# moritzmeister/hops-examples

Hardware: AMD Instinct MI355X
Metric: images/sec MNIST CNN + steps/sec Chicago-taxi DNN at 1/2/4/8 MI355X (higher is better)
Workload: dtype bf16; 1 GPU; model=MNIST CNN (experiment.mirrored model, 1394282 params), Adadelta(1.0), global_batch=32, per_gpu_batch=32, parallelism=dp1, engine=PersistentMnistStep, hipgraph=False, steps_per_execution=32, warmup_steps_run=5

## Files before the change

csrc/ops/mnist_persist.hip:

```cpp
#include "common.h"
#include "mnist_cnn.h"
#include "optim_core.h"
#include "wg_prims.h"

namespace mnistp {
using namespace wgp;
using namespace mnist_cnn;

constexpr int B = 32;
constexpr int NCONV = C2 * 128 + C2 + C1 * 4 + C1;
constexpr int OFF_B2 = C2 * 128, OFF_W1 = OFF_B2 + C2, OFF_B1 = OFF_W1 + C1 * 4;
constexpr int SLICE = 52, NSLICE = (NCONV + SLICE - 1) / SLICE;
constexpr int NRED = 19;
constexpr int NHEAD = B;
constexpr int GRID = NPOS + NHEAD;
constexpr int PAY = 272;
constexpr int PAY_DH = 0, PAY_H = 128, PAY_DL = 256, PAY_LOSS = 268, PAY_COR = 269;
constexpr int FL_A = 0, FL_B = 256, FL_C = 512, FL_D = 768, FL_WORDS = 1024;
constexpr int FL_EPOCH = FL_WORDS - 2;
constexpr int D_F32 = OFF_B2 * 2;
constexpr int D_BYTES = D_F32 + (NCONV - OFF_B2) * 4;
constexpr int TGB_N = NHEAD * (HID / 2);
constexpr int TG_WORDS = 2 * 2 * TGB_N;
static_assert(FL_WORDS % 2 == 0 && TGB_N % 256 == 0, "granules are 8-B aligned; every thread owns TGB_N / 256");

constexpr int DHS = row_stride(HID), DCS = row_stride(4 * B);
static_assert(DHS == 136 && DCS == 136, "strides the kernel was tuned with");

constexpr int L_W1 = 0;
constexpr int L_W2 = L_W1 + HID * W1S * 2;
constexpr int L_CW1 = L_W2 + C2 * W2S * 2;
constexpr int L_CB1 = L_CW1 + C1 * 4 * 4;
constexpr int L_CB2 = L_CB1 + C1 * 4;
constexpr int L_XIN = L_CB2 + C2 * 4;
constexpr int L_C1 = L_XIN + B * 16 * 4;
constexpr int L_POOL = L_C1 + B * 9 * C1S * 2;
constexpr int L_AM = L_POOL + B * PLS * 2;
constexpr int L_DH = L_AM + B * C2;
constexpr int L_DC2 = L_DH + B * DHS * 2;
constexpr int L_STG = L_DC2 + C2 * DCS * 2;
constexpr int L_RED = L_STG + NCONV * 4;
constexpr int L_SL = L_RED + 1024 * 4;
constexpr int L_KEEP = L_SL + 3 * 64 * 4;
constexpr int LDS_BYTES = L_KEEP + B * C2;

constexpr int H_W2 = 0;
constexpr int H_B2 = H_W2 + 3 * NCLS * HID * 4;
constexpr int H_B1 = H_B2 + 3 * 16 * 4;
constexpr int H_RED = H_B1 + 3 * HID * 4;
constexpr int H_H = H_RED + 8 * HID * 4;
constexpr int H_LOG = H_H + HID * 4;
constexpr int H_PAY = H_LOG + 16 * 4;
constexpr int H_ALL = H_PAY + PAY * 4;
constexpr int H_END = H_ALL + NHEAD * PAY * 4;
constexpr int H_DHS = H_END;
static_assert(H_DHS + B * DHS * 2 <= LDS_BYTES, "head LDS map must fit the position map");

constexpr int XMAX = 8;
constexpr long XS_POOL = (long)NPOS * 4 * 64 * 16;
constexpr long XS_DHT = 8L * 64 * 16;
constexpr int NFC2 = NCLS * HID + HID + NCLS, NFC2P = 1424;
constexpr long XS_FC2 = NFC2P * 4;
constexpr long XS_CONV = (long)NSLICE * SLICE * 4;
constexpr long XO_POOL = 0, XO_DHT = XO_POOL + 2L * XMAX * XS_POOL, XO_FC2 = XO_DHT + 2L * XMAX * XS_DHT,
               XO_CONV = XO_FC2 + 2L * XMAX * XS_FC2, X_BYTES = XO_CONV + 2L * XMAX * XS_CONV;
constexpr int XF_POOL = 0, XF_H = XMAX * NPOS, XF_CONV = XF_H + XMAX, XF_WORDS = XF_CONV + XMAX * NSLICE;
static_assert(NFC2 <= NFC2P && NFC2P % 4 == 0 && X_BYTES < 0x7fffffffL, "exchange geometry");
static_assert(LDS_BYTES <= 160 * 1024, "one workgroup per CU: 160 KiB LDS");
static_assert(L_RED + NRED * SLICE * 4 <= L_SL && 2 * 32 * 5 * 4 <= 1024 * 4, "reduce scratch");
static_assert(NRED * 13 <= 256 && NSLICE * SLICE >= NCONV && NSLICE <= NPOS, "slice geometry");

struct Args {
  float* master;
  bf16_raw* shadow;
  float* s1;
  float* s2;
  long off[8];
  const unsigned char* xs;
  const long long* ys;
  long nbatch;
  long long* cursor;
  unsigned long long* rng;
  float* step_dev;
  const float* hp_dev;
  float* slabA;
  float* slabB;
  float* slabC;
  float* slabD;
  unsigned* flags;
  unsigned* err;
  float* out;
  unsigned long long* dbg;
  OptHP hp;
  float drop_p, xscale, xshift;
  unsigned salt;
  int nsteps;
  int acquire;
  long long tmo;
  long long tmo0;
  int pollw, stagger;
  int pollw_a, pollw_b, pollw_c, pollw_d;
  int head1w;
  int hand;
  float inv_gb;
  int world, rank;
  int loopback;
  int xfence;
  long long* xstep;
  unsigned char* xbuf[XMAX];
  unsigned* xflag[XMAX];
};


__device__ __forceinline__ int xslot(const Args& a, int peer) { return a.loopback ? peer : a.rank; }

__device__ __forceinline__ bool wait_all(const unsigned* flags, int n, unsigned epoch, unsigned* err, unsigned code,
                                      int acquire, int* s_ok, long long tmo, int pollw = 1, int stagger = 0,
                                      int poll1 = 0) {
  if (pollw <= 1) {
    if (threadIdx.x < 64) {
      const int lane = threadIdx.x;
      int good = 1;
      const long long t0 = wall_clock64();
      for (unsigned spins = 0;; ++spins) {
        int ok = 1;
        unsigned e = poll1 ? flag_load(err) : 0u;
        for (int k = lane; k < n; k += 64) ok &= flag_load(flags + k) == epoch;
        if (__all(ok)) break;
        if (!poll1) e = flag_load(err);
        if (__builtin_amdgcn_readfirstlane(e) != 0u) {
          good = 0;
          break;
        }
        if ((spins & 15u) == 15u && wall_clock64() - t0 > tmo) {
          if (lane == 0) atomicCAS(err, 0u, code);
          good = 0;
          break;
        }
        __builtin_amdgcn_s_sleep(1);
      }
      if (acquire && good) __builtin_amdgcn_fence(__ATOMIC_ACQUIRE, "agent");
      drain();
      if (lane == 0) *s_ok = good;
    }
    __syncthreads();
    const int g = *s_ok;
    return g != 0;
  }
  volatile int* gen = s_ok + 1;
  const int wave = threadIdx.x >> 6;
  if (wave < pollw) {
    const int lane = threadIdx.x & 63;
    int good = 1;
    for (int d = 0; d < wave * stagger && __builtin_amdgcn_readfirstlane(*gen) != (int)code; ++d)
      __builtin_amdgcn_s_sleep(1);
    const long long t0 = wall_clock64();
    for (unsigned spins = 0;; ++spins) {
      if (__builtin_amdgcn_readfirstlane(*gen) == (int)code) break;
      int ok = 1;
      unsigned e = poll1 ? flag_load(err) : 0u;
      for (int k = lane; k < n; k += 64) ok &= flag_load(flags + k) == epoch;
      if (__all(ok)) {
        if (lane == 0) {
          s_ok[0] = 1;
          *gen = (int)code;
        }
        break;
      }
      if (!poll1) e = flag_load(err);
      if (__builtin_amdgcn_readfirstlane(e) != 0u) good = 0;
      if ((spins & 15u) == 15u && wall_clock64() - t0 > tmo) {
        if (lane == 0) atomicCAS(err, 0u, code);
        good = 0;
      }
      if (!good) {
        if (lane == 0) {
          s_ok[0] = 0;
          *gen = (int)code;
        }
        break;
      }
      __builtin_amdgcn_s_sleep(1);
    }
    if (acquire) __builtin_amdgcn_fence(__ATOMIC_ACQUIRE, "agent");
    drain();
  }
  __syncthreads();
  const int g = s_ok[0];
  return g != 0;
}

__device__ __forceinline__ bool wait_peers(const Args& a, int base, int stride, unsigned epoch, unsigned code,
                                        int* s_ok) {
  if (threadIdx.x < 64) {
    const int lane = threadIdx.x;
    const unsigned* page = a.xflag[a.rank];
    int good = 1;
    const long long t0 = wall_clock64();
    for (unsigned spins = 0;; ++spins) {
      const bool mine = lane < a.world && lane != a.rank;
      unsigned e = (a.hand & 2) ? flag_load(a.err) : 0u;
      const int ok = !mine || (int)(xflag_load(page + base + lane * stride) - epoch) >= 0;
      if (__all(ok)) break;
      if (!(a.hand & 2)) e = flag_load(a.err);
      if (__builtin_amdgcn_readfirstlane(e) != 0u) {
        good = 0;
        break;
      }
      if ((spins & 15u) == 15u && wall_clock64() - t0 > a.tmo) {
        if (lane == 0) atomicCAS(a.err, 0u, code);
        good = 0;
        break;
      }
      __builtin_amdgcn_s_sleep(1);
    }
    drain();
    if (lane == 0) *s_ok = good;
  }
  __syncthreads();
  const int g = *s_ok;
  return g != 0;
}
__device__ __forceinline__ void raise_peers(const Args& a, int base, int stride, unsigned epoch) {
// ... 460 lines not shown
      for (int j = 0; j < 8; ++j) acc[j] = (f32x4){0.f, 0.f, 0.f, 0.f};
      const bf16_raw* cb = C1 + (2 * fq * 9 + (tq >> 1) * 3 + (tq & 1)) * C1S + 4 * tp;
      bf16x8 af[2], bfr[2][8];
      auto cfrag = [&](int kk, int st) {
#pragma unroll
        for (int j = 0; j < 8; ++j) {
          const int t = j >> 1;
          const bf16_raw* q = cb + (kk * 8 * 9 + (t >> 1) * 3 + (t & 1)) * C1S + (j & 1) * 16;
          bfr[st][j] = lds_tr(q, q + 9 * C1S);
        }
      };
      auto afrag = [&](int kk, int st) { af[st] = lds8(DC2 + (w * 16 + fr) * DCS + kk * 32 + fq * 8); };
      cfrag(0, 0);
      __syncthreads();
      stamp(a, s, 4);
      afrag(0, 0);
#pragma unroll
      for (int kk = 0; kk < 4; ++kk) {
        if (kk + 1 < 4) {
          afrag(kk + 1, (kk + 1) & 1);
          cfrag(kk + 1, (kk + 1) & 1);
        }
        __builtin_amdgcn_sched_barrier(0);
#pragma unroll
        for (int j = 0; j < 8; ++j) acc[j] = mma32(af[kk & 1], bfr[kk & 1][j], acc[j]);
      }
#pragma unroll
      for (int j = 0; j < 8; ++j)
#pragma unroll
        for (int r = 0; r < 4; ++r) STG[(w * 16 + fq * 4 + r) * 128 + j * 16 + fr] = acc[j][r];
    }
    {
      const int mh = w >> 1, h = w & 1, ci = h * 16 + fr;
      bf16x8 af[2][4], bfr[2][4];
#pragma unroll
      for (int kk = 0; kk < 2; ++kk) {
        const int k1 = kk * 32 + 8 * fq + tq;
#pragma unroll
        for (int i = 0; i < 4; ++i) {
          const int m0 = (mh * 4 + i) * 16 + 4 * tp;
          af[kk][i] = lds_tr(DC2 + k1 * DCS + m0, DC2 + (k1 + 4) * DCS + m0);
        }
#pragma unroll
        for (int t = 0; t < 4; ++t) {
          const int c0 = (2 * t + h) * 16 + 4 * tp;
          bfr[kk][t] = lds_tr(W2 + k1 * W2S + c0, W2 + (k1 + 4) * W2S + c0);
        }
      }
      __syncthreads();
      {
        const auto R = rsrc(a.slabC + ((long)par * NPOS + p) * NCONV);
        constexpr int NK = OFF_B2 / 4 / 256;
        f32x4 v[NK];
#pragma unroll
        for (int k = 0; k < NK; ++k) v[k] = *(const f32x4*)(STG + (tid + 256 * k) * 4);
        __builtin_amdgcn_sched_barrier(0);
#pragma unroll
        for (int k = 0; k < NK; ++k) bst16<SC1>(R, (tid + 256 * k) * 16, v[k]);
      }
      f32x4 acc[4][4];
#pragma unroll
      for (int i = 0; i < 4; ++i)
#pragma unroll
        for (int t = 0; t < 4; ++t) acc[i][t] = (f32x4){0.f, 0.f, 0.f, 0.f};
#pragma unroll
      for (int kk = 0; kk < 2; ++kk)
#pragma unroll
        for (int t = 0; t < 4; ++t)
#pragma unroll
          for (int i = 0; i < 4; ++i) acc[i][t] = mma32(af[kk][i], bfr[kk][t], acc[i][t]);
      bf16_raw c1v[4][9];
#pragma unroll
      for (int i = 0; i < 4; ++i)
#pragma unroll
        for (int pos = 0; pos < 9; ++pos) c1v[i][pos] = C1[((4 * (mh * 4 + i) + fq) * 9 + pos) * C1S + ci];
      if constexpr (!DP) {
        bf16x8 wa[2], wb[4];
#pragma unroll
        for (int ii = 0; ii < 2; ++ii) {
          const int n0 = (2 * w + ii) * 16 + 4 * tp;
          wa[ii] = lds_tr(DH + (8 * fq + tq) * DHS + n0, DH + (8 * fq + tq + 4) * DHS + n0);
        }
#pragma unroll
        for (int j = 0; j < 4; ++j) {
          const int c0 = j * 16 + 4 * tp;
          wb[j] = lds_tr(POOL + (8 * fq + tq) * PLS + c0, POOL + (8 * fq + tq + 4) * PLS + c0);
        }
#pragma unroll
        for (int ii = 0; ii < 2; ++ii)
#pragma unroll
          for (int j = 0; j < 4; ++j) gw[ii][j] = mma32(wa[ii], wb[j], (f32x4){0.f, 0.f, 0.f, 0.f});
      }
      float gk[5] = {0.f, 0.f, 0.f, 0.f, 0.f};
      f32x4 xq[2][4];
#pragma unroll
      for (int c = 0; c < 4; ++c) xq[0][c] = *(const f32x4*)(XIN + (4 * (mh * 4) + fq) * 16 + 4 * c);
#pragma unroll
      for (int i = 0; i < 4; ++i) {
        if (i + 1 < 4) {
#pragma unroll
          for (int c = 0; c < 4; ++c) xq[(i + 1) & 1][c] = *(const f32x4*)(XIN + (4 * (mh * 4 + i + 1) + fq) * 16 + 4 * c);
        }
        float d[9];
#pragma unroll
        for (int k = 0; k < 9; ++k) d[k] = 0.f;
#pragma unroll
        for (int t = 0; t < 4; ++t)
#pragma unroll
          for (int q = 0; q < 4; ++q) d[((q >> 1) + (t >> 1)) * 3 + (q & 1) + (t & 1)] += acc[i][t][q];
        const f32x4* xi = xq[i & 1];
#pragma unroll
        for (int py = 0; py < 3; ++py)
#pragma unroll
          for (int px = 0; px < 3; ++px) {
            const int pos = py * 3 + px;
            const float dd = (short)c1v[i][pos] > 0 ? d[pos] : 0.f;
            gk[0] = fmaf(dd, xi[py][px], gk[0]);
            gk[1] = fmaf(dd, xi[py][px + 1], gk[1]);
            gk[2] = fmaf(dd, xi[py + 1][px], gk[2]);
            gk[3] = fmaf(dd, xi[py + 1][px + 1], gk[3]);
            gk[4] += dd;
          }
      }
#pragma unroll
      for (int k = 0; k < 5; ++k) {
        gk[k] += __shfl_xor(gk[k], 16, 64);
        gk[k] += __shfl_xor(gk[k], 32, 64);
      }
      if (fq == 0) {
#pragma unroll
        for (int k = 0; k < 5; ++k) RED[(mh * 32 + ci) * 5 + k] = gk[k];
      }
    }
    __syncthreads();
    if (tid < 32 * 5) {
      const int ci = tid / 5, k = tid - ci * 5;
      const float v = RED[ci * 5 + k] + RED[(32 + ci) * 5 + k];
      if (k < 4) STG[OFF_W1 + ci * 4 + k] = v;
      else STG[OFF_B1 + ci] = v;
    }
    __syncthreads();
    stamp(a, s, 5);
    {
      const auto R = rsrc(a.slabC + ((long)par * NPOS + p) * NCONV);
      const int idx = OFF_B2 / 4 + tid;
      if (idx < NCONV / 4) bst16<SC1>(R, idx * 16, *(const f32x4*)(STG + idx * 4));
      drain();
      __syncthreads();
      if (tid == 0) flag_store(a.flags + FL_C + p, ep);
    }
    stamp(a, s, 6);
    if (owner) {
      const int e0 = p * SLICE;
      constexpr int NKC = (NPOS + NRED - 1) / NRED;
      static_assert(6 * NKC <= 64, "the flags of a wave's groups (64 threads span at most 6 groups of 13): one per lane");
      if ((a.hand & 8) && !a.acquire) {
        const int j = tid % 13, g = tid / 13;
        const bool act = g < NRED && e0 + 4 * j < NCONV;
        const int g0 = (w * 64) / 13, g1 = (w * 64 + 63) / 13;
        const int lg = g0 + lane / NKC, lp = lg + NRED * (lane % NKC);
        const bool mine = lane < 6 * NKC && lg <= g1 && lg < NRED && lp < NPOS;
        const auto R = rsrc(a.slabC + (long)par * NPOS * NCONV);
        f32x4 v[NKC];
#pragma unroll
        for (int k = 0; k < NKC; ++k) v[k] = (f32x4){0.f, 0.f, 0.f, 0.f};
        const unsigned pend = !act ? 0u : (g + NRED * (NKC - 1) < NPOS ? (1u << NKC) - 1u : (1u << (NKC - 1)) - 1u);
        gather_rows<NKC>(a.flags + FL_C + lp, mine, act ? (g - g0) * NKC : 0, pend, ep, a.err, ecode(3, s), s_ok + 2,
                         a.tmo, [&](int k) { v[k] = bld16<SC1>(R, ((g + NRED * k) * NCONV + e0 + 4 * j) * 4); });
        stamp(a, s, 7);
#pragma unroll
        for (int k = 0; k < NKC; ++k) asm volatile("" ::"v"(v[k]));
        if (g < NRED) {
          f32x4 acc = (f32x4){0.f, 0.f, 0.f, 0.f};
#pragma unroll
          for (int k = 0; k < NKC; ++k) acc += v[k];
          *(f32x4*)(RED + g * SLICE + 4 * j) = acc;
        }
        __syncthreads();
        const int f = s_ok[2];
        if (f) return;
      } else {
      if (!wait_all(a.flags + FL_C, NPOS, ep, a.err, ecode(3, s), a.acquire, s_ok, a.tmo, a.pollw_c, a.stagger, (a.hand & 2)))
        return;
      stamp(a, s, 7);
      if (tid < 13 * NRED) {
        const int j = tid % 13, g = tid / 13;
        f32x4 acc = (f32x4){0.f, 0.f, 0.f, 0.f};
        if (e0 + 4 * j < NCONV) {
          const auto R = rsrc(a.slabC + (long)par * NPOS * NCONV);
          constexpr int NK = (NPOS + NRED - 1) / NRED;
          f32x4 v[NK];
#pragma unroll
          for (int k = 0; k < NK; ++k) {
            const int pp = g + NRED * k;
            v[k] = pp < NPOS ? bld16<SC1>(R, (pp * NCONV + e0 + 4 * j) * 4) : (f32x4){0.f, 0.f, 0.f, 0.f};
          }
#pragma unroll
          for (int k = 0; k < NK; ++k) acc += v[k];
        }
        *(f32x4*)(RED + g * SLICE + 4 * j) = acc;
      }
      __syncthreads();
      }
      const int e = e0 + tid;
      float gs = 0.f;
      if (tid < SLICE) {
        for (int g = 0; g < NRED; ++g) gs += RED[g * SLICE + tid];
      }
      if constexpr (DP) {
        if (tid < 64) {
          if (tid < SLICE) {
            for (int r = 0; r < a.world; ++r) {
              if (r == a.rank) continue;
              bst4<SYS>(rsrc(a.xbuf[r] + XO_CONV + (par * XMAX + xslot(a, r)) * XS_CONV), e * 4, gs);
            }
          }
          drain();
          raise_peers(a, XF_CONV + p, NSLICE, gep);
        }
        if (!wait_peers(a, XF_CONV + p, NSLICE, gep, ecode(6, s), s_ok)) return;
        if (tid < SLICE) {
          const auto X = rsrc(a.xbuf[a.rank] + XO_CONV + (long)par * XMAX * XS_CONV);
          float v[XMAX];
#pragma unroll
          for (int r = 0; r < XMAX; ++r) v[r] = r < a.world && r != a.rank ? bld4<SYS>(X, (int)(r * XS_CONV) + e * 4) : gs;
          float t = 0.f;
#pragma unroll
          for (int r = 0; r < XMAX; ++r)
            if (r < a.world) t += v[r];
          gs = t;
        }
      }
      if (tid < SLICE) {
        float wn = 0.f;
        if (e < NCONV) {
          SLm[tid] = adadelta(SLm[tid], gs * hp.gscale, SL1[tid], SL2[tid], hp);
          wn = SLm[tid];
        }
        const float wnext = __shfl_down(wn, 1, 64);
        unsigned char* D = (unsigned char*)a.slabD + (long)par * D_BYTES;
        if (e < OFF_B2) {
          if (!(tid & 1))
            __hip_atomic_store((gu32*)(D + e * 2), (unsigned)f2bf_hw(wn) | ((unsigned)f2bf_hw(wnext) << 16),
                               __ATOMIC_RELAXED, __HIP_MEMORY_SCOPE_AGENT);
        } else if (e < NCONV) {
          __hip_atomic_store((gu32*)(D + D_F32 + (e - OFF_B2) * 4), __float_as_uint(wn), __ATOMIC_RELAXED,
                             __HIP_MEMORY_SCOPE_AGENT);
        }
      }
      if (w == 0) {
        drain();
        if (lane == 0) flag_store(a.flags + FL_D + p, ep);
      }
      stamp(a, s, 8);
    }
    if constexpr (DP) {
      if (!wait_peers(a, XF_H, 1, gep, ecode(7, s), s_ok)) return;
      if (!wait_peers(a, XF_POOL + p, NPOS, gep, ecode(8, s), s_ok)) return;
#pragma unroll
      for (int ii = 0; ii < 2; ++ii)
#pragma unroll
        for (int j = 0; j < 4; ++j) gw[ii][j] = (f32x4){0.f, 0.f, 0.f, 0.f};
      const auto XP = rsrc(a.xbuf[a.rank] + XO_POOL + (long)par * XMAX * XS_POOL + (long)p * 4096);
      const auto XD = rsrc(a.xbuf[a.rank] + XO_DHT + (long)par * XMAX * XS_DHT);
      constexpr int PF = 3;
      bf16x8 af[PF][2], bfr[PF][4];
      auto fetch = [&](int r, int b) {
        if (r == a.rank) {
#pragma unroll
          for (int ii = 0; ii < 2; ++ii) {
            const int n0 = (2 * w + ii) * 16 + 4 * tp;
            af[b][ii] = lds_tr(DH + (8 * fq + tq) * DHS + n0, DH + (8 * fq + tq + 4) * DHS + n0);
          }
#pragma unroll
          for (int j = 0; j < 4; ++j) {
            const int c0 = j * 16 + 4 * tp;
            bfr[b][j] = lds_tr(POOL + (8 * fq + tq) * PLS + c0, POOL + (8 * fq + tq + 4) * PLS + c0);
          }
        } else {
#pragma unroll
          for (int ii = 0; ii < 2; ++ii)
            af[b][ii] = __builtin_bit_cast(bf16x8, bld16<SYS>(XD, (int)(r * XS_DHT) + ((2 * w + ii) * 64 + lane) * 16));
#pragma unroll
          for (int j = 0; j < 4; ++j)
            bfr[b][j] = __builtin_bit_cast(bf16x8, bld16<SYS>(XP, (int)(r * XS_POOL) + (j * 64 + lane) * 16));
        }
      };
#pragma unroll
      for (int r = 0; r < PF - 1; ++r)
        if (r < a.world) fetch(r, r);
#pragma unroll
      for (int r = 0; r < XMAX; ++r) {
        if (r < a.world) {
          if (r + PF - 1 < XMAX && r + PF - 1 < a.world) fetch(r + PF - 1, (r + PF - 1) % PF);
#pragma unroll
          for (int ii = 0; ii < 2; ++ii)
#pragma unroll
            for (int j = 0; j < 4; ++j)
              gw[ii][j] += mma32(af[r % PF][ii], bfr[r % PF][j], (f32x4){0.f, 0.f, 0.f, 0.f});
        }
      }
    }
#pragma unroll
    for (int ii = 0; ii < 2; ++ii)
#pragma unroll
      for (int j = 0; j < 4; ++j)
#pragma unroll
        for (int r = 0; r < 4; ++r) {
          wm[ii][j][r] = adadelta(wm[ii][j][r], gw[ii][j][r] * hp.gscale, g1[ii][j][r], g2[ii][j][r], hp);
          W1[((2 * w + ii) * 16 + fq * 4 + r) * W1S + j * 16 + fr] = f2bf_hw(wm[ii][j][r]);
        }
    if (s + 1 < a.nsteps) draw_keep(s + 1);
    stamp(a, s, 9);
    if (!wait_all(a.flags + FL_D, NSLICE, ep, a.err, ecode(4, s), a.acquire, s_ok, a.tmo, a.pollw_d, a.stagger,
                  (a.hand & 2)))
      return;
    stamp(a, s, 10);
    {
      const auto R = rsrc((const unsigned char*)a.slabD + (long)par * D_BYTES);
      constexpr int NB = OFF_B2 * 2 / 16;
      constexpr int NF = (NCONV - OFF_B2) / 4;
      f32x4 dv[NB / 256 + 1];
#pragma unroll
      for (int k = 0; k < NB / 256; ++k) dv[k] = bld16<SC1>(R, (tid + 256 * k) * 16);
      dv[NB / 256] = tid < NF ? bld16<SC1>(R, D_F32 + tid * 16) : (f32x4){0.f, 0.f, 0.f, 0.f};
#pragma unroll
      for (int k = 0; k < NB / 256; ++k) {
        const int c = tid + 256 * k;
        *(f32x4*)(W2 + (c >> 4) * W2S + (c & 15) * 8) = dv[k];
      }
      if (tid < NF) {
        const int j = OFF_B2 + tid * 4;
        float* dst = j < OFF_W1 ? CB2 + (j - OFF_B2) : (j < OFF_B1 ? CW1 + (j - OFF_W1) : CB1 + (j - OFF_B1));
        *(f32x4*)dst = dv[NB / 256];
      }
    }
    __syncthreads();
    stamp(a, s, 11);
  }

#pragma unroll
  for (int ii = 0; ii < 2; ++ii)
#pragma unroll
    for (int j = 0; j < 4; ++j)
#pragma unroll
      for (int r = 0; r < 4; ++r) {
        const int n = (2 * w + ii) * 16 + fq * 4 + r, co = j * 16 + fr;
        const long ai = a.off[4] + (long)n * KIN + p * C2 + co;
        a.master[ai] = wm[ii][j][r];
        a.s1[ai] = g1[ii][j][r];
        a.s2[ai] = g2[ii][j][r];
        a.shadow[ai] = f2bf_hw(wm[ii][j][r]);
      }
  if (owner && tid < SLICE) {
    const int e = p * SLICE + tid;
    if (e < NCONV) {
      const long ci = conv_idx(a, e);
      a.master[ci] = SLm[tid];
      a.s1[ci] = SL1[tid];
      a.s2[ci] = SL2[tid];
      a.shadow[ci] = f2bf_hw(SLm[tid]);
    }
  }
  stamp(a, a.nsteps - 1, 14);
  if (p == 0 && tid == 0) {
    if constexpr (DP) a.xstep[0] = xs0 + a.nsteps;
    a.cursor[0] = (cur0 + a.nsteps) % a.nbatch;
    *(unsigned long long*)(a.flags + FL_EPOCH) = eb + (unsigned long long)a.nsteps;
    a.rng[1] = ctr0 + (unsigned long long)a.nsteps;
    if (a.step_dev) a.step_dev[0] += (float)a.nsteps;
  }
}

template <bool DP>
__device__ __forceinline__ void head_wg(const Args& a, unsigned char* smem, int* s_ok, const OptHP& hp,
                                        long long cur0, long long xs0, unsigned long long eb) {
  const int i = blockIdx.x - NPOS;
  const int tid = threadIdx.x, lane = tid & 63;
  float* HW = (float*)(smem + H_W2);
  float* HW1 = HW + NCLS * HID;
  float* HW2 = HW1 + NCLS * HID;
  float* HB2 = (float*)(smem + H_B2);
  float* HB1 = (float*)(smem + H_B1);
  float* RED = (float*)(smem + H_RED);
  float* HH = (float*)(smem + H_H);
  float* LOG = (float*)(smem + H_LOG);
  float* PAYL = (float*)(smem + H_PAY);
  float* ALL = (float*)(smem + H_ALL);
  {
    constexpr int NJ = NCLS * HID / 256;
    float v0[NJ], v1[NJ], v2[NJ];
#pragma unroll
    for (int q = 0; q < NJ; ++q) {
      const long ai = a.off[6] + tid + 256 * q;
      v0[q] = a.master[ai];
      v1[q] = a.s1[ai];
      v2[q] = a.s2[ai];
    }
#pragma unroll
    for (int q = 0; q < NJ; ++q) {
      HW[tid + 256 * q] = v0[q];
      HW1[tid + 256 * q] = v1[q];
      HW2[tid + 256 * q] = v2[q];
    }
  }
  if (tid < NCLS) {
    const long ai = a.off[7] + tid;
    HB2[tid] = a.master[ai];
    HB2[16 + tid] = a.s1[ai];
    HB2[32 + tid] = a.s2[ai];
  }
  if (tid < HID) {
    const long ai = a.off[5] + tid;
    HB1[tid] = a.master[ai];
    HB1[128 + tid] = a.s1[ai];
    HB1[256 + tid] = a.s2[ai];
  }
  if (tid == 0) {
    PAYL[266] = PAYL[267] = PAYL[270] = PAYL[271] = 0.f;
  }
  __syncthreads();

  for (int s = 0; s < a.nsteps; ++s) {
    const unsigned ep = (unsigned)(eb + (unsigned long long)s + 1ull);
    const int par = s & 1;
    const int y = (int)a.ys[((cur0 + s) % a.nbatch) * B + i];
    if (!wait_all(a.flags + FL_A, NPOS, ep, a.err, s ? ecode(1, s) : ecode(12, 0), a.acquire, s_ok,
                  s ? a.tmo : a.tmo0, a.pollw_a, a.stagger, (a.hand & 2)))
      return;
    stamp(a, s, 0);
    {
      const int n4 = tid & 31, g = tid >> 5;
      const auto R = rsrc(a.slabA + (long)par * NPOS * B * HID);
      constexpr int NK = (NPOS + 7) / 8;
      f32x4 v[NK];
#pragma unroll
      for (int k = 0; k < NK; ++k) {
        const int pp = g + 8 * k;
        v[k] = pp < NPOS ? bld16<SC1>(R, ((pp * B + i) * HID + n4 * 4) * 4) : (f32x4){0.f, 0.f, 0.f, 0.f};
      }
      f32x4 acc = v[0];
#pragma unroll
      for (int k = 1; k < NK; ++k) acc += v[k];
      *(f32x4*)(RED + g * HID + n4 * 4) = acc;
    }
    __syncthreads();
    if (a.head1w) {
      if (tid < 64) {
        const int n0 = 2 * lane;
        float h[2];
#pragma unroll
        for (int u = 0; u < 2; ++u) {
          float v = 0.f;
#pragma unroll
          for (int g = 0; g < 8; ++g) v += RED[g * HID + n0 + u];
          h[u] = fmaxf(v + HB1[n0 + u], 0.f);
        }
        float z[NCLS];
#pragma unroll
        for (int c = 0; c < NCLS; ++c)
          z[c] = wave_sum(fmaf(h[1], HW[c * HID + n0 + 1], h[0] * HW[c * HID + n0])) + HB2[c];
        float m = z[0];
#pragma unroll
        for (int c = 1; c < NCLS; ++c) m = fmaxf(m, z[c]);
        float e[NCLS], se = 0.f, zy = 0.f;
        int am = NCLS;
// ... 125 lines not shown
#pragma unroll 8
      for (int b = 0; b < B; ++b) gl[NW] += ALL[b * PAY + PAY_DH + tid];
    }
    if (tid < NCLS) {
      for (int b = 0; b < B; ++b) gl[NW + 1] += ALL[b * PAY + PAY_DL + tid];
    }
    if constexpr (DP) {
      const unsigned gep = (unsigned)(xs0 + s + 1);
      if (i == 0) {
        bf16_raw* DS = (bf16_raw*)(smem + H_DHS);
        for (int e = tid; e < B * HID; e += 256) DS[(e >> 7) * DHS + (e & 127)] = f2bf_hw(ALL[(e >> 7) * PAY + PAY_DH + (e & 127)]);
        __syncthreads();
        const int w = tid >> 6, fr = lane & 15, fq = lane >> 4, tq = fr >> 2, tp = fr & 3;
        f32x4 fd[2];
#pragma unroll
        for (int ii = 0; ii < 2; ++ii) {
          const int n0 = (2 * w + ii) * 16 + 4 * tp;
          fd[ii] = __builtin_bit_cast(f32x4, lds_tr(DS + (8 * fq + tq) * DHS + n0, DS + (8 * fq + tq + 4) * DHS + n0));
        }
        for (int r = 0; r < a.world; ++r) {
          if (r == a.rank) continue;
          const int sl = xslot(a, r);
          const auto XG = rsrc(a.xbuf[r] + XO_FC2 + (par * XMAX + sl) * XS_FC2);
#pragma unroll
          for (int k = 0; k < NW; ++k) bst4<SYS>(XG, (tid + 256 * k) * 4, gl[k]);
          if (tid < HID) bst4<SYS>(XG, (NCLS * HID + tid) * 4, gl[NW]);
          if (tid < NCLS) bst4<SYS>(XG, (NCLS * HID + HID + tid) * 4, gl[NW + 1]);
          const auto XD = rsrc(a.xbuf[r] + XO_DHT + (par * XMAX + sl) * XS_DHT);
#pragma unroll
          for (int ii = 0; ii < 2; ++ii) bst16<SYS>(XD, ((2 * w + ii) * 64 + lane) * 16, fd[ii]);
        }
        drain();
        __syncthreads();
        if (tid < 64) raise_peers(a, XF_H, 1, gep);
      }
      if (!wait_peers(a, XF_H, 1, gep, ecode(9, s), s_ok)) return;
      const auto X = rsrc(a.xbuf[a.rank] + XO_FC2 + (long)par * XMAX * XS_FC2);
      float t[NW + 2];
#pragma unroll
      for (int k = 0; k < NW + 2; ++k) t[k] = 0.f;
      float v[XMAX][NW + 2];
#pragma unroll
      for (int r = 0; r < XMAX; ++r) {
        const bool peer = r < a.world && r != a.rank;
        const int o = (int)(r * XS_FC2);
#pragma unroll
        for (int k = 0; k < NW; ++k) v[r][k] = peer ? bld4<SYS>(X, o + (tid + 256 * k) * 4) : gl[k];
        v[r][NW] = peer && tid < HID ? bld4<SYS>(X, o + (NCLS * HID + tid) * 4) : gl[NW];
        v[r][NW + 1] = peer && tid < NCLS ? bld4<SYS>(X, o + (NCLS * HID + HID + tid) * 4) : gl[NW + 1];
      }
#pragma unroll
      for (int r = 0; r < XMAX; ++r)
        if (r < a.world) {
#pragma unroll
          for (int k = 0; k < NW + 2; ++k) t[k] += v[r][k];
        }
#pragma unroll
      for (int k = 0; k < NW + 2; ++k) gl[k] = t[k];
    }
#pragma unroll
    for (int k = 0; k < NW; ++k) {
      const int j = tid + 256 * k;
      HW[j] = adadelta(HW[j], gl[k] * hp.gscale, HW1[j], HW2[j], hp);
    }
    if (tid < HID) HB1[tid] = adadelta(HB1[tid], gl[NW] * hp.gscale, HB1[128 + tid], HB1[256 + tid], hp);
    if (tid < NCLS) HB2[tid] = adadelta(HB2[tid], gl[NW + 1] * hp.gscale, HB2[16 + tid], HB2[32 + tid], hp);
    if (i == 0 && tid == 255) {
      float l = 0.f, cc = 0.f;
      for (int b = 0; b < B; ++b) {
        l += ALL[b * PAY + PAY_LOSS];
        cc += ALL[b * PAY + PAY_COR];
      }
      a.out[2 * s] = l * (1.f / B);
      a.out[2 * s + 1] = cc;
    }
    __syncthreads();
    stamp(a, s, 2);
  }
  if (i == 0) {
    for (int j = tid; j < NCLS * HID; j += 256) {
      const long ai = a.off[6] + j;
      a.master[ai] = HW[j];
      a.s1[ai] = HW1[j];
      a.s2[ai] = HW2[j];
      a.shadow[ai] = f2bf_hw(HW[j]);
    }
    if (tid < NCLS) {
      const long ai = a.off[7] + tid;
      a.master[ai] = HB2[tid];
      a.s1[ai] = HB2[16 + tid];
      a.s2[ai] = HB2[32 + tid];
      a.shadow[ai] = f2bf_hw(HB2[tid]);
    }
    if (tid < HID) {
      const long ai = a.off[5] + tid;
      a.master[ai] = HB1[tid];
      a.s1[ai] = HB1[128 + tid];
      a.s2[ai] = HB1[256 + tid];
      a.shadow[ai] = f2bf_hw(HB1[tid]);
    }
  }
}

template <bool DP>
__global__ __launch_bounds__(256, 1) void mnist_persist_k(const Args a) {
  extern __shared__ __attribute__((aligned(16))) unsigned char smem[];
  __shared__ int s_ok[3];
  stamp(a, 0, 13);
  if (threadIdx.x == 0) s_ok[0] = s_ok[1] = s_ok[2] = 0;
  const OptHP hp = load_hp(a.hp, a.hp_dev);
  const long long cur0 = a.cursor[0];
  const long long xs0 = DP ? a.xstep[0] : 0;
  const unsigned long long eb = *(const unsigned long long*)(a.flags + FL_EPOCH);
  if (blockIdx.x < NPOS) {
    position_wg<DP>(a, smem, s_ok, hp, cur0, a.rng[0], a.rng[1], xs0, eb);
  } else {
    head_wg<DP>(a, smem, s_ok, hp, cur0, xs0, eb);
  }
}

}

static int g_persist_reload = 0;
extern "C" void hopsx_mnist_persist_reload_knobs() { g_persist_reload = 1; }

extern "C" int hopsx_mnist_persist(const uint64_t* p, int np, const long* iv, int ni, const float* fv, int nf,
                                   hipStream_t st) {
  using namespace mnistp;
  if (np < 18 || ni < 18 || nf < 8) return (int)hipErrorInvalidValue;
  if (iv[11] != B || iv[10] < 1 || iv[8] < 1) return (int)hipErrorInvalidValue;
  const int world = (int)iv[13], rank = (int)iv[14];
  if (world < 1 || world > XMAX || rank < 0 || rank >= world) return (int)hipErrorInvalidValue;
  const bool dp = world > 1;
  if (dp && np < 19 + 2 * world) return (int)hipErrorInvalidValue;
  Args a{};
  a.master = (float*)p[0];
  a.shadow = (bf16_raw*)p[1];
  a.s1 = (float*)p[2];
  a.s2 = (float*)p[3];
  a.xs = (const unsigned char*)p[4];
  a.ys = (const long long*)p[5];
  a.cursor = (long long*)p[6];
  a.rng = (unsigned long long*)p[7];
  a.step_dev = (float*)p[8];
  a.hp_dev = (const float*)p[9];
  a.slabA = (float*)p[10];
  a.slabB = (float*)p[11];
  a.slabC = (float*)p[12];
  a.slabD = (float*)p[13];
  a.flags = (unsigned*)p[14];
  a.err = (unsigned*)p[15];
  a.out = (float*)p[16];
  a.dbg = (unsigned long long*)p[17];
  for (int k = 0; k < 8; ++k) a.off[k] = iv[k];
  a.nbatch = iv[8];
  a.salt = (unsigned)iv[9];
  a.nsteps = (int)iv[10];
  a.acquire = (int)iv[12];
  a.world = world;
  a.rank = rank;
  a.loopback = (int)iv[15];
  a.xfence = (int)iv[17];
  a.tmo = (long long)iv[16] * 100000ll;
  a.tmo0 = a.tmo;
  static int kn_ok = 0, kn_pollw, kn_stagger, kn_a, kn_b, kn_c, kn_d, kn_head1w, kn_memset, kn_coop;
  static int kn_tagged, kn_gate, kn_poll1, kn_prog;
  static long kn_start_ms;
  if (!kn_ok || g_persist_reload) {
    auto pw = [&](const char* name, long dflt) {
      const long v = hopsx_env_int(name, dflt);
      return (int)(v >= 1 && v <= 4 ? v : 1);
    };
    kn_pollw = pw("HOPSX_PERSIST_POLLW", 1);
    kn_stagger = (int)hopsx_env_int("HOPSX_PERSIST_STAGGER", 12);
    kn_a = pw("HOPSX_PERSIST_POLLW_A", kn_pollw);
    kn_b = pw("HOPSX_PERSIST_POLLW_B", kn_pollw);
    kn_c = pw("HOPSX_PERSIST_POLLW_C", 4);
    kn_d = pw("HOPSX_PERSIST_POLLW_D", kn_pollw);
    kn_head1w = (int)hopsx_env_int("HOPSX_PERSIST_HEAD1W", 1);
    kn_memset = (int)hopsx_env_int("HOPSX_PERSIST_MEMSET", 0);
    kn_coop = (int)hopsx_env_int("HOPSX_PERSIST_COOP", 0);
    kn_start_ms = hopsx_env_int("HOPSX_PERSIST_START_MS", 50);
    kn_tagged = hopsx_env_int("HOPSX_PERSIST_TAGGED", 1) != 0;
    const long gt = hopsx_env_int("HOPSX_PERSIST_GATE", NHEAD / 2);
    kn_gate = (int)(gt >= 1 && gt <= NHEAD ? gt : NHEAD / 2);
    kn_poll1 = hopsx_env_int("HOPSX_PERSIST_POLL1", 1) != 0;
    kn_prog = (int)(hopsx_env_int("HOPSX_PERSIST_PROG", 3) & 2);
    kn_ok = 1;
    g_persist_reload = 0;
  }
  a.pollw = kn_pollw;
  a.stagger = kn_stagger;
  a.pollw_a = kn_a;
  a.pollw_b = kn_b;
  a.pollw_c = kn_c;
  a.pollw_d = kn_d;
  a.head1w = kn_head1w;
  a.hand = kn_tagged | (kn_poll1 << 1) | (kn_prog << 2) | (kn_gate << 8);
  if (kn_start_ms > 0 && kn_start_ms * 100000ll < a.tmo) a.tmo0 = kn_start_ms * 100000ll;
  a.inv_gb = 1.f / (float)(world * B);
  if (dp) {
    a.xstep = (long long*)p[18];
    for (int r = 0; r < world; ++r) {
      a.xbuf[r] = (unsigned char*)p[19 + r];
      a.xflag[r] = (unsigned*)p[19 + world + r];
      if (!a.xbuf[r] || !a.xflag[r] || ((uint64_t)a.xbuf[r] & 15)) return (int)hipErrorInvalidValue;
    }
  }
  a.drop_p = fv[0];
  a.xscale = fv[1];
  a.xshift = fv[2];
  a.hp = OptHP{fv[3], fv[4], fv[5], fv[6], fv[7], 0.f, 0.f, 0.f};
  static bool attr[2] = {false, false};
  const void* fn = dp ? (const void*)mnist_persist_k<true> : (const void*)mnist_persist_k<false>;
  if (!attr[dp]) {
    const hipError_t e = hipFuncSetAttribute(fn, hipFuncAttributeMaxDynamicSharedMemorySize, LDS_BYTES);
    if (e != hipSuccess) return (int)e;
    attr[dp] = true;
  }
  if (kn_memset) {
    const hipError_t e = hipMemsetAsync(a.flags, 0, FL_WORDS * sizeof(unsigned), st);
    if (e != hipSuccess) return (int)e;
  }
  if (kn_coop) {
    void* kargs[] = {(void*)&a};
    const hipError_t e = hipLaunchCooperativeKernel(fn, dim3(GRID), dim3(256), kargs, LDS_BYTES, st);
    if (e != hipSuccess) {
      (void)hipGetLastError();
      return (int)e;
    }
    return (int)hipSuccess;
  }
  if (dp)
    hipLaunchKernelGGL(mnist_persist_k<true>, dim3(GRID), dim3(256), LDS_BYTES, st, a);
  else
    hipLaunchKernelGGL(mnist_persist_k<false>, dim3(GRID), dim3(256), LDS_BYTES, st, a);
  return (int)hipGetLastError();
}

extern "C" int hopsx_mnist_persist_occupancy(int dp) {
  using namespace mnistp;
  const void* fn = dp ? (const void*)mnist_persist_k<true> : (const void*)mnist_persist_k<false>;
  if (hipFuncSetAttribute(fn, hipFuncAttributeMaxDynamicSharedMemorySize, LDS_BYTES) != hipSuccess) return -1;
  int n = 0;
  if (hipOccupancyMaxActiveBlocksPerMultiprocessor(&n, fn, 256, LDS_BYTES) != hipSuccess) return -1;
  return n;
}

extern "C" void hopsx_mnist_persist_geom(long* g) {
  using namespace mnistp;
  g[0] = B;
  g[1] = NPOS;
  g[2] = NHEAD;
  g[3] = GRID;
  g[4] = NCONV;
  g[5] = NSLICE;
  g[6] = SLICE;
  g[7] = PAY;
  g[8] = FL_WORDS;
  g[9] = LDS_BYTES;
  g[10] = D_BYTES;
  g[11] = X_BYTES;
  g[12] = XF_WORDS;
  g[13] = XMAX;
  g[14] = XO_POOL;
  g[15] = XS_POOL;
  g[16] = XO_DHT;
  g[17] = XS_DHT;
  g[18] = XO_FC2;
  g[19] = XS_FC2;
  g[20] = XO_CONV;
  g[21] = XS_CONV;
  g[22] = TG_WORDS;
}
```

Measured before the change: 1.411 million images/sec.

## Widen conv-gradient slices to one wave with aligned 128-byte rows

```diff
diff --git a/csrc/ops/mnist_persist.hip b/csrc/ops/mnist_persist.hip
--- a/csrc/ops/mnist_persist.hip
+++ b/csrc/ops/mnist_persist.hip
@@ -10,8 +10,10 @@
 constexpr int B = 32;
 constexpr int NCONV = C2 * 128 + C2 + C1 * 4 + C1;
 constexpr int OFF_B2 = C2 * 128, OFF_W1 = OFF_B2 + C2, OFF_B1 = OFF_W1 + C1 * 4;
-constexpr int SLICE = 52, NSLICE = (NCONV + SLICE - 1) / SLICE;
+constexpr int SLICE = 64, NSLICE = (NCONV + SLICE - 1) / SLICE;
 constexpr int NRED = 19;
+constexpr int NKC = (NPOS + NRED - 1) / NRED;
+constexpr int NQ = SLICE / 4;
 constexpr int NHEAD = B;
 constexpr int GRID = NPOS + NHEAD;
 constexpr int PAY = 272;
@@ -40,7 +42,7 @@
 constexpr int L_DC2 = L_DH + B * DHS * 2;
 constexpr int L_STG = L_DC2 + C2 * DCS * 2;
 constexpr int L_RED = L_STG + NCONV * 4;
-constexpr int L_SL = L_RED + 1024 * 4;
+constexpr int L_SL = L_RED + NRED * SLICE * 4;
 constexpr int L_KEEP = L_SL + 3 * 64 * 4;
 constexpr int LDS_BYTES = L_KEEP + B * C2;
 
@@ -67,8 +69,12 @@
 constexpr int XF_POOL = 0, XF_H = XMAX * NPOS, XF_CONV = XF_H + XMAX, XF_WORDS = XF_CONV + XMAX * NSLICE;
 static_assert(NFC2 <= NFC2P && NFC2P % 4 == 0 && X_BYTES < 0x7fffffffL, "exchange geometry");
 static_assert(LDS_BYTES <= 160 * 1024, "one workgroup per CU: 160 KiB LDS");
-static_assert(L_RED + NRED * SLICE * 4 <= L_SL && 2 * 32 * 5 * 4 <= 1024 * 4, "reduce scratch");
-static_assert(NRED * 13 <= 256 && NSLICE * SLICE >= NCONV && NSLICE <= NPOS, "slice geometry");
+static_assert(L_RED + NRED * SLICE * 4 <= L_SL && 2 * 32 * 5 * 4 <= NRED * SLICE * 4, "reduce scratch");
+static_assert(SLICE * 4 % 128 == 0 && NCONV * 4 % 128 == 0, "a slice row is whole 128-byte lines of an aligned slabC row");
+static_assert(OFF_B2 % SLICE == 0 && D_F32 % 128 == 0 && D_BYTES % 128 == 0, "no slice straddles the bf16 / fp32 parts of D");
+static_assert(NSLICE * SLICE >= NCONV && NSLICE <= NPOS && SLICE == 64, "slice geometry: one wave updates a slice");
+static_assert(NQ == 16 && NRED > 16 && NRED - 16 <= 3 && 5 * NKC <= 64 && 2 * NKC <= 32 && NRED * (NKC - 1) < NPOS,
+              "gather geometry: at most 5 groups' flags per wave, one per lane; both items' rows in one pend mask");
 
 struct Args {
   float* master;
@@ -835,55 +841,50 @@
     stamp(a, s, 6);
     if (owner) {
       const int e0 = p * SLICE;
-      constexpr int NKC = (NPOS + NRED - 1) / NRED;
-      static_assert(6 * NKC <= 64, "the flags of a wave's groups (64 threads span at most 6 groups of 13): one per lane");
+      const int j = lane & (NQ - 1), lq = lane >> 4, g = 4 * w + lq, gx = 16 + w;
+      const bool act = e0 + 4 * j < NCONV, two = lq == 3 && gx < NRED;
+      const auto R = rsrc(a.slabC + (long)par * NPOS * NCONV);
+      f32x4 v[2 * NKC];
+#pragma unroll
+      for (int k = 0; k < 2 * NKC; ++k) v[k] = (f32x4){0.f, 0.f, 0.f, 0.f};
+      auto load = [&](int k) {
+        const int pp = k < NKC ? g + NRED * k : gx + NRED * (k - NKC);
+        v[k] = bld16<SC1>(R, (pp * NCONV + e0 + 4 * j) * 4);
+      };
+      const unsigned rows2 = gx + NRED * (NKC - 1) < NPOS ? (1u << NKC) - 1u : (1u << (NKC - 1)) - 1u;
+      const unsigned pend = !act ? 0u : ((1u << NKC) - 1u) | (two ? rows2 << NKC : 0u);
+      bool lost = false;
       if ((a.hand & 8) && !a.acquire) {
-        const int j = tid % 13, g = tid / 13;
-        const bool act = g < NRED && e0 + 4 * j < NCONV;
-        const int g0 = (w * 64) / 13, g1 = (w * 64 + 63) / 13;
-        const int lg = g0 + lane / NKC, lp = lg + NRED * (lane % NKC);
-        const bool mine = lane < 6 * NKC && lg <= g1 && lg < NRED && lp < NPOS;
-        const auto R = rsrc(a.slabC + (long)par * NPOS * NCONV);
-        f32x4 v[NKC];
-#pragma unroll
-        for (int k = 0; k < NKC; ++k) v[k] = (f32x4){0.f, 0.f, 0.f, 0.f};
-        const unsigned pend = !act ? 0u : (g + NRED * (NKC - 1) < NPOS ? (1u << NKC) - 1u : (1u << (NKC - 1)) - 1u);
-        gather_rows<NKC>(a.flags + FL_C + lp, mine, act ? (g - g0) * NKC : 0, pend, ep, a.err, ecode(3, s), s_ok + 2,
-                         a.tmo, [&](int k) { v[k] = bld16<SC1>(R, ((g + NRED * k) * NCONV + e0 + 4 * j) * 4); });
+        const int lp = lane < 4 * NKC ? 4 * w + lane / NKC + NRED * (lane % NKC) : gx + NRED * (lane - 4 * NKC);
+        const bool mine = lane < 4 * NKC || (gx < NRED && lane < 5 * NKC && lp < NPOS);
+        gather_rows<2 * NKC>(a.flags + FL_C + lp, mine, lq * NKC, pend, ep, a.err, ecode(3, s), s_ok + 2, a.tmo, load);
         stamp(a, s, 7);
-#pragma unroll
-        for (int k = 0; k < NKC; ++k) asm volatile("" ::"v"(v[k]));
-        if (g < NRED) {
-          f32x4 acc = (f32x4){0.f, 0.f, 0.f, 0.f};
-#pragma unroll
-          for (int k = 0; k < NKC; ++k) acc += v[k];
-          *(f32x4*)(RED + g * SLICE + 4 * j) = acc;
-        }
-        __syncthreads();
+      } else {
+        lost = !wait_all(a.flags + FL_C, NPOS, ep, a.err, ecode(3, s), a.acquire, s_ok, a.tmo, a.pollw_c, a.stagger,
+                         (a.hand & 2));
+        stamp(a, s, 7);
+#pragma unroll
+        for (int k = 0; k < 2 * NKC; ++k)
+          if (!lost && ((pend >> k) & 1u)) load(k);
+      }
+#pragma unroll
+      for (int k = 0; k < 2 * NKC; ++k) asm volatile("" ::"v"(v[k]));
+      {
+        f32x4 acc = (f32x4){0.f, 0.f, 0.f, 0.f};
+#pragma unroll
+        for (int k = 0; k < NKC; ++k) acc += v[k];
+        *(f32x4*)(RED + g * SLICE + 4 * j) = acc;
+      }
+      if (two) {
+        f32x4 acc = (f32x4){0.f, 0.f, 0.f, 0.f};
+#pragma unroll
+        for (int k = 0; k < NKC; ++k) acc += v[NKC + k];
+        *(f32x4*)(RED + gx * SLICE + 4 * j) = acc;
+      }
+      __syncthreads();
+      {
         const int f = s_ok[2];
-        if (f) return;
-      } else {
-      if (!wait_all(a.flags + FL_C, NPOS, ep, a.err, ecode(3, s), a.acquire, s_ok, a.tmo, a.pollw_c, a.stagger, (a.hand & 2)))
-        return;
-      stamp(a, s, 7);
-      if (tid < 13 * NRED) {
-        const int j = tid % 13, g = tid / 13;
-        f32x4 acc = (f32x4){0.f, 0.f, 0.f, 0.f};
-        if (e0 + 4 * j < NCONV) {
-          const auto R = rsrc(a.slabC + (long)par * NPOS * NCONV);
-          constexpr int NK = (NPOS + NRED - 1) / NRED;
-          f32x4 v[NK];
-#pragma unroll
-          for (int k = 0; k < NK; ++k) {
-            const int pp = g + NRED * k;
-            v[k] = pp < NPOS ? bld16<SC1>(R, (pp * NCONV + e0 + 4 * j) * 4) : (f32x4){0.f, 0.f, 0.f, 0.f};
-          }
-#pragma unroll
-          for (int k = 0; k < NK; ++k) acc += v[k];
-        }
-        *(f32x4*)(RED + g * SLICE + 4 * j) = acc;
-      }
-      __syncthreads();
+        if (lost || f) return;
       }
       const int e = e0 + tid;
       float gs = 0.f;
@@ -914,7 +915,7 @@
           gs = t;
         }
       }
-      if (tid < SLICE) {
+      if (w == 0) {
         float wn = 0.f;
         if (e < NCONV) {
           SLm[tid] = adadelta(SLm[tid], gs * hp.gscale, SL1[tid], SL2[tid], hp);
@@ -922,16 +923,14 @@
         }
         const float wnext = __shfl_down(wn, 1, 64);
         unsigned char* D = (unsigned char*)a.slabD + (long)par * D_BYTES;
-        if (e < OFF_B2) {
-          if (!(tid & 1))
+        if (p < OFF_B2 / SLICE) {
+          if (!(lane & 1))
             __hip_atomic_store((gu32*)(D + e * 2), (unsigned)f2bf_hw(wn) | ((unsigned)f2bf_hw(wnext) << 16),
                                __ATOMIC_RELAXED, __HIP_MEMORY_SCOPE_AGENT);
         } else if (e < NCONV) {
           __hip_atomic_store((gu32*)(D + D_F32 + (e - OFF_B2) * 4), __float_as_uint(wn), __ATOMIC_RELAXED,
                              __HIP_MEMORY_SCOPE_AGENT);
         }
-      }
-      if (w == 0) {
         drain();
         if (lane == 0) flag_store(a.flags + FL_D + p, ep);
       }
@@ -995,6 +994,16 @@
         }
     if (s + 1 < a.nsteps) draw_keep(s + 1);
     stamp(a, s, 9);
+    if (!owner && tid < 64) {
+      constexpr int G0 = OFF_B2 / SLICE;
+      const bool mine = lane < NSLICE - G0;
+      const long long t0 = wall_clock64();
+      for (;;) {
+        const unsigned f = mine ? flag_load(a.flags + FL_D + G0 + lane) : ep;
+        if (__all(f == ep) || wall_clock64() - t0 > 2000) break;
+        __builtin_amdgcn_s_sleep(4);
+      }
+    }
     if (!wait_all(a.flags + FL_D, NSLICE, ep, a.err, ecode(4, s), a.acquire, s_ok, a.tmo, a.pollw_d, a.stagger,
                   (a.hand & 2)))
       return;
@@ -1426,6 +1435,7 @@
   a.err = (unsigned*)p[15];
   a.out = (float*)p[16];
   a.dbg = (unsigned long long*)p[17];
+  if (((uint64_t)a.slabC & 127) || ((uint64_t)a.slabD & 127)) return (int)hipErrorInvalidValue;
   for (int k = 0; k < 8; ++k) a.off[k] = iv[k];
   a.nbatch = iv[8];
   a.salt = (unsigned)iv[9];
```

New measurement: 1.439 million images/sec (median of 6 runs). +2.0%, better.
